# cyoq/onitama-alphazero

Hardware: AMD Instinct MI355X
Metric: MCTS node-expansions/sec/GPU @400 sims; self-play games/sec at 1/2/4/8 GPU (higher is better)
Workload: dtype fp32 (fp16x3 split)

## Files before the change

onitama-alphazero_amd/csrc/oaz_device.h:

```cpp
#pragma once

#include <stdint.h>

#include "../../include/onitama_az.h"

#if defined(__HIPCC__)
#include <hip/hip_runtime.h>
#define OAZ_HD __host__ __device__ __forceinline__
#else
#define OAZ_HD inline
#endif

namespace oaz {

constexpr uint32_t kCardPos[16] = {0x20004000u, 0x0440A000u, 0x02202000u, 0x00828000u,
                                   0x01220000u, 0x02940000u, 0x02142000u, 0x00948000u,
                                   0x0280A000u, 0x02804000u, 0x0100A000u, 0x01104000u,
                                   0x01044000u, 0x01140000u, 0x02048000u, 0x00902000u};
constexpr uint32_t kCardMir[16] = {0x01000200u, 0x02811000u, 0x02022000u, 0x00A08000u,
                                   0x00224000u, 0x0014A000u, 0x02142000u, 0x00948000u,
                                   0x0280A000u, 0x0100A000u, 0x02804000u, 0x01044000u,
                                   0x01104000u, 0x00144000u, 0x00902000u, 0x02048000u};
constexpr uint8_t kCardColor[16] = {1, 0, 0, 0, 1, 0, 1, 0, 1, 0, 1, 0, 1, 0, 1, 0};

constexpr uint32_t kRedKingStart = 0x00000200u;
constexpr uint32_t kBlueKingStart = 0x20000000u;
constexpr uint32_t kBluePawnsStart = 0xD8000000u;
constexpr uint32_t kRedPawnsStart = 0x00000D80u;
constexpr int kBlueTemple = 2;
constexpr int kRedTemple = 22;

OAZ_HD constexpr uint32_t sq_bit(int sq) { return 0x80000000u >> sq; }

struct AttackTable {
    uint32_t m[2][16][25];
};

constexpr AttackTable make_attack_table() {
    AttackTable t{};
    for (int color = 0; color < 2; ++color)
        for (int card = 0; card < 16; ++card) {
            const uint32_t pat = color ? kCardMir[card] : kCardPos[card];
            for (int from = 0; from < 25; ++from) {
                uint32_t m = 0;
                for (int j = 0; j < 25; ++j) {
                    if (!(pat & sq_bit(j))) continue;
                    const int dr = j / 5 - 2, dc = j % 5 - 2;
                    const int r = from / 5 + dr, c = from % 5 + dc;
                    if (r >= 0 && r < 5 && c >= 0 && c < 5) m |= sq_bit(r * 5 + c);
                }
                t.m[color][card][from] = m;
            }
        }
    return t;
}

constexpr AttackTable kAttackHost = make_attack_table();

OAZ_HD bool is_win(int r) { return r == OAZ_RED_WIN || r == OAZ_BLUE_WIN; }

OAZ_HD int make_move(oaz_state& s, int from, int to, int piece, int slot, int color) {
    const uint32_t fb = sq_bit(from), tb = sq_bit(to);
    const int enemy = color ^ 1;
    if (piece == OAZ_PAWN) s.pawns[color] &= ~fb;
    else s.kings[color] &= ~fb;
    int res = OAZ_IN_PROGRESS;
    if (s.pawns[enemy] & tb) {
        s.pawns[enemy] &= ~tb;
        res = OAZ_CAPTURE;
    } else if (s.kings[enemy] & tb) {
        s.kings[enemy] &= ~tb;
        res = color == OAZ_RED ? OAZ_RED_WIN : OAZ_BLUE_WIN;
    }
    if (piece == OAZ_PAWN) s.pawns[color] |= tb;
    else s.kings[color] |= tb;
    if (piece == OAZ_KING && to == (color == OAZ_RED ? kBlueTemple : kRedTemple))
        res = color == OAZ_RED ? OAZ_RED_WIN : OAZ_BLUE_WIN;
    if (slot < 4) {
        const uint8_t t = s.cards[slot];
        s.cards[slot] = s.cards[4];
        s.cards[4] = t;
    }
    return res;
}

OAZ_HD int state_card(const oaz_state& s, int i) {
    uint32_t w;
    __builtin_memcpy(&w, s.cards, 4);
    return i < 4 ? (int)((w >> (8 * i)) & 0xFFu) : (int)s.cards[4];
}
OAZ_HD void state_rotate(oaz_state& s, int slot) {
    uint32_t w;
    __builtin_memcpy(&w, s.cards, 4);
    const uint32_t sh = 8u * (uint32_t)slot;
    const uint8_t t = (uint8_t)(w >> sh);
    w = (w & ~(0xFFu << sh)) | ((uint32_t)s.cards[4] << sh);
    __builtin_memcpy(s.cards, &w, 4);
    s.cards[4] = t;
}
OAZ_HD int make_move_regs(oaz_state& s, int from, int to, int piece, int slot, int color) {
    const uint32_t fb = sq_bit(from), tb = sq_bit(to);
    const bool blue = color != OAZ_RED;
    uint32_t mp = blue ? s.pawns[1] : s.pawns[0], mk = blue ? s.kings[1] : s.kings[0];
    uint32_t ep = blue ? s.pawns[0] : s.pawns[1], ek = blue ? s.kings[0] : s.kings[1];
    if (piece == OAZ_PAWN) mp &= ~fb;
    else mk &= ~fb;
    int res = OAZ_IN_PROGRESS;
    if (ep & tb) {
        ep &= ~tb;
        res = OAZ_CAPTURE;
    } else if (ek & tb) {
        ek &= ~tb;
        res = color == OAZ_RED ? OAZ_RED_WIN : OAZ_BLUE_WIN;
    }
    if (piece == OAZ_PAWN) mp |= tb;
    else mk |= tb;
    if (piece == OAZ_KING && to == (color == OAZ_RED ? kBlueTemple : kRedTemple))
        res = color == OAZ_RED ? OAZ_RED_WIN : OAZ_BLUE_WIN;
    s.pawns[0] = blue ? ep : mp;
    s.pawns[1] = blue ? mp : ep;
    s.kings[0] = blue ? ek : mk;
    s.kings[1] = blue ? mk : ek;
    if (slot < 4) state_rotate(s, slot);
    return res;
}

OAZ_HD int current_state(const oaz_state& s) {
    if (s.kings[0] == 0 || s.kings[1] == kRedKingStart) return OAZ_BLUE_WIN;
    if (s.kings[1] == 0 || s.kings[0] == kBlueKingStart) return OAZ_RED_WIN;
    return OAZ_IN_PROGRESS;
}

OAZ_HD double reward(int result, int color) {
    if (!is_win(result)) return 0.0;
    return ((result == OAZ_RED_WIN) == (color == OAZ_RED)) ? 1.0 : -1.0;
}

OAZ_HD void initial_state(const uint8_t deck[5], oaz_state& s) {
    s.kings[0] = kRedKingStart;
    s.kings[1] = kBlueKingStart;
    s.pawns[0] = kRedPawnsStart;
    s.pawns[1] = kBluePawnsStart;
    for (int i = 0; i < 5; ++i) s.cards[i] = deck[i];
    s.to_move = kCardColor[deck[4] & 15];
    s.pad[0] = s.pad[1] = 0;
}

OAZ_HD uint16_t pack_move(int from, int to, int slot, int piece) {
    return (uint16_t)(from | (to << 5) | (slot << 10) | (piece << 12));
}
OAZ_HD int mv_from(uint32_t m) { return m & 31; }
OAZ_HD int mv_to(uint32_t m) { return (m >> 5) & 31; }
OAZ_HD int mv_slot(uint32_t m) { return (m >> 10) & 3; }
OAZ_HD int mv_piece(uint32_t m) { return (m >> 12) & 1; }

struct u32x4 {
    uint32_t x, y, z, w;
};

OAZ_HD u32x4 philox(uint64_t key, uint32_t c0, uint32_t c1, uint32_t c2, uint32_t c3) {
    uint32_t k0 = (uint32_t)key, k1 = (uint32_t)(key >> 32);
#if defined(__HIP_DEVICE_COMPILE__)
#pragma unroll
#endif
    for (int r = 0; r < 10; ++r) {
        const uint64_t p0 = (uint64_t)0xD2511F53u * c0;
        const uint64_t p1 = (uint64_t)0xCD9E8D57u * c2;
        const uint32_t n0 = (uint32_t)(p1 >> 32) ^ c1 ^ k0;
        const uint32_t n2 = (uint32_t)(p0 >> 32) ^ c3 ^ k1;
        c1 = (uint32_t)p1;
        c3 = (uint32_t)p0;
        c0 = n0;
        c2 = n2;
        k0 += 0x9E3779B9u;
        k1 += 0xBB67AE85u;
    }
    return {c0, c1, c2, c3};
}

OAZ_HD double u01(uint32_t a, uint32_t b) {
    const uint64_t m = ((uint64_t)(a >> 5) << 26) | (uint64_t)(b >> 6);
    return ((double)m + 0.5) * (1.0 / 9007199254740992.0);
}

#ifndef OAZ_NOISE_F32
#define OAZ_NOISE_F32 0
#endif
#if OAZ_NOISE_F32
typedef float noise_t;
#else
typedef double noise_t;
#endif

OAZ_HD float nz_u(uint32_t x) {
    return (float)(((x >> 9) << 1) | 1u) * (1.0f / 16777216.0f);
}
OAZ_HD float nz_log(float x) {
    uint32_t b = __builtin_bit_cast(uint32_t, x);
    int e = (int)((b >> 23) & 0xFF) - 127;
    b = (b & 0x007FFFFFu) | 0x3F800000u;
    float m = __builtin_bit_cast(float, b);
    if (m > 1.41421356f) {
        m = m * 0.5f;
        e += 1;
    }
    const float t = (m - 1.0f) / (m + 1.0f), t2 = t * t;
    const float p = t * (2.0f + t2 * (0.666666667f + t2 * (0.4f + t2 * (0.285714286f + t2 * 0.222222222f))));
    return (float)e * 0.693147182f + p;
}
OAZ_HD float nz_exp(float x) {
    if (x < -87.0f) return 0.0f;
    if (x > 88.0f) return __builtin_bit_cast(float, 0x7F800000u);
    const float k = (float)(int)(x * 1.44269504f + (x >= 0.0f ? 0.5f : -0.5f));
    const float r = (x - k * 0.693145752f) - k * 1.42860677e-6f;
    const float q = 1.0f + r * (1.0f + r * (0.5f + r * (0.166666667f + r * (0.0416666667f + r * (0.00833333333f +
                                                                                        r * 0.00138888889f)))));
    return q * __builtin_bit_cast(float, (uint32_t)((int)k + 127) << 23);
}
OAZ_HD float root_noise_f32(uint64_t seed, uint64_t game, uint32_t c2, uint32_t idx, float alpha, int K) {
    const float ia = 1.0f / alpha, ib = 1.0f / (alpha * (float)(K - 1));
    for (uint32_t t = 0; t < 1024u; ++t) {
        const u32x4 r = philox(seed, (uint32_t)game, (uint32_t)(game >> 32), c2, (idx << 12) | t);
        const float lx = nz_log(nz_u(r.x)) * ia, ly = nz_log(nz_u(r.y)) * ib;
        if (nz_exp(lx) + nz_exp(ly) <= 1.0f) return 1.0f / (1.0f + nz_exp(ly - lx));
        const float lx2 = nz_log(nz_u(r.z)) * ia, ly2 = nz_log(nz_u(r.w)) * ib;
        if (nz_exp(lx2) + nz_exp(ly2) <= 1.0f) return 1.0f / (1.0f + nz_exp(ly2 - lx2));
    }
    return 1.0f / (float)K;
}

constexpr double kLn2Hi = 6.93147180369123816490e-01, kLn2Lo = 1.90821492927058770002e-10;
OAZ_HD double nz_fma(double a, double b, double c) { return __builtin_fma(a, b, c); }
OAZ_HD double nz_log64(double x) {
    uint64_t b = __builtin_bit_cast(uint64_t, x);
    int e = (int)((b >> 52) & 0x7FF) - 1023;
    double m = __builtin_bit_cast(double, (b & 0x000FFFFFFFFFFFFFull) | 0x3FF0000000000000ull);
    if (m > 1.4142135623730951) {
        m = m * 0.5;
        e += 1;
    }
    const double t = (m - 1.0) / (m + 1.0), t2 = t * t;
    double p = 2.0 / 21.0;
    p = nz_fma(p, t2, 2.0 / 19.0);
    p = nz_fma(p, t2, 2.0 / 17.0);
    p = nz_fma(p, t2, 2.0 / 15.0);
    p = nz_fma(p, t2, 2.0 / 13.0);
    p = nz_fma(p, t2, 2.0 / 11.0);
    p = nz_fma(p, t2, 2.0 / 9.0);
    p = nz_fma(p, t2, 2.0 / 7.0);
    p = nz_fma(p, t2, 2.0 / 5.0);
    p = nz_fma(p, t2, 2.0 / 3.0);
    p = nz_fma(p * t2, t, 2.0 * t);
    const double de = (double)e;
    return nz_fma(de, kLn2Hi, nz_fma(de, kLn2Lo, p));
}
OAZ_HD double nz_exp64(double x) {
    if (x < -708.0) return 0.0;
    if (x > 709.0) return __builtin_bit_cast(double, 0x7FF0000000000000ull);
    const double k = (double)(int)(x * 1.4426950408889634 + (x >= 0.0 ? 0.5 : -0.5));
    const double r = (x - k * kLn2Hi) - k * kLn2Lo;
    double q = 1.0 / 6227020800.0;
    q = nz_fma(q, r, 1.0 / 479001600.0);
    q = nz_fma(q, r, 1.0 / 39916800.0);
    q = nz_fma(q, r, 1.0 / 3628800.0);
    q = nz_fma(q, r, 1.0 / 362880.0);
    q = nz_fma(q, r, 1.0 / 40320.0);
    q = nz_fma(q, r, 1.0 / 5040.0);
    q = nz_fma(q, r, 1.0 / 720.0);
    q = nz_fma(q, r, 1.0 / 120.0);
    q = nz_fma(q, r, 1.0 / 24.0);
    q = nz_fma(q, r, 1.0 / 6.0);
    q = nz_fma(q, r, 0.5);
    q = nz_fma(q, r, 1.0);
    q = nz_fma(q, r, 1.0);
    return q * __builtin_bit_cast(double, (uint64_t)((int64_t)k + 1023) << 52);
}
OAZ_HD double root_noise_f64(uint64_t seed, uint64_t game, uint32_t c2, uint32_t idx, double alpha, int K) {
    const double ia = 1.0 / alpha, ib = 1.0 / (alpha * (double)(K - 1));
    for (uint32_t t = 0; t < 2048u; ++t) {
        const u32x4 r = philox(seed, (uint32_t)game, (uint32_t)(game >> 32), c2, (idx << 12) | t);
        const double lx = nz_log64(u01(r.x, r.y)) * ia, ly = nz_log64(u01(r.z, r.w)) * ib;
        const double x = nz_exp64(lx), y = nz_exp64(ly), sum = x + y;
        if (sum <= 1.0) return (x > 0.0 && y > 0.0) ? x / sum : 1.0 / (1.0 + nz_exp64(ly - lx));
    }
    return 1.0 / (double)K;
}
OAZ_HD noise_t root_noise(uint64_t seed, uint64_t game, uint32_t c2, uint32_t idx, double alpha, int K) {
#if OAZ_NOISE_F32
    return root_noise_f32(seed, game, c2, idx, (float)alpha, K);
#else
    return root_noise_f64(seed, game, c2, idx, alpha, K);
#endif
}

OAZ_HD void deal_deck(uint64_t seed, uint64_t game_id, uint8_t out[5]) {
    uint8_t cards[16];
    for (int i = 0; i < 16; ++i) cards[i] = (uint8_t)i;
    uint32_t w[16];
    for (uint32_t q = 0; q < 4; ++q) {
        const u32x4 r = philox(seed, (uint32_t)game_id, (uint32_t)(game_id >> 32), 0xDEA1u, q);
        w[4 * q] = r.x;
        w[4 * q + 1] = r.y;
        w[4 * q + 2] = r.z;
        w[4 * q + 3] = r.w;
    }
    for (int i = 15, k = 0; i >= 1; --i, ++k) {
        const uint32_t j = (uint32_t)(((uint64_t)w[k] * (uint64_t)(i + 1)) >> 32);
        const uint8_t t = cards[i];
        cards[i] = cards[j];
        cards[j] = t;
    }
    for (int i = 0; i < 5; ++i) out[i] = cards[i];
}

OAZ_HD uint64_t slot_game_id(uint64_t seq, uint32_t world, uint32_t rank, uint32_t G, uint32_t g) {
    return (seq * (uint64_t)world + (uint64_t)rank) * (uint64_t)G + (uint64_t)g;
}

OAZ_HD uint64_t splitmix64(uint64_t x) {
    uint64_t z = x + 0x9E3779B97F4A7C15ull;
    z = (z ^ (z >> 30)) * 0xBF58476D1CE4E5B9ull;
    z = (z ^ (z >> 27)) * 0x94D049BB133111EBull;
    return z ^ (z >> 31);
}

OAZ_HD uint64_t hash_state(const oaz_state& s) {
    uint64_t h = splitmix64((uint64_t)s.kings[0] | ((uint64_t)s.kings[1] << 32));
    h = splitmix64(h ^ ((uint64_t)s.pawns[0] | ((uint64_t)s.pawns[1] << 32)));
    const uint64_t c = (uint64_t)(s.cards[0] & 15) | ((uint64_t)(s.cards[1] & 15) << 4) |
                       ((uint64_t)(s.cards[2] & 15) << 8) | ((uint64_t)(s.cards[3] & 15) << 12) |
                       ((uint64_t)(s.cards[4] & 15) << 16) | ((uint64_t)(s.to_move & 1) << 20);
    return splitmix64(h ^ c);
}
OAZ_HD float hash_policy(uint64_t h, int i) {
    return (float)((splitmix64(h + (uint64_t)i) >> 40) + 1) * (1.0f / 16777216.0f);
}
OAZ_HD float hash_value(uint64_t h) {
    const int32_t v = (int32_t)(splitmix64(h ^ 0x5DEECE66Dull) >> 40) - 8388608;
    return (float)v * (1.0f / 8388608.0f);
}

OAZ_HD int ab_msb_pos(uint32_t v) { return v ? 32 - __builtin_ctz(v) : 0; }
OAZ_HD int ab_distance(int from, int to) {
    const int dx = to / 5 - from / 5, dy = to % 5 - from % 5, d2 = dx * dx + dy * dy;
    return (d2 >= 1) + (d2 >= 4) + (d2 >= 9) + (d2 >= 16) + (d2 >= 25) + (d2 >= 36);
}
OAZ_HD int ab_pst_sum(uint32_t p) {
    constexpr uint32_t kRow = 0xF8000000u, kCol = 0x84210800u;
    constexpr uint32_t r13 = (kRow >> 5) | (kRow >> 15), r2 = kRow >> 10, c13 = (kCol >> 1) | (kCol >> 3), c2 = kCol >> 2;
    return 4 * (__builtin_popcount(p & r13) + 2 * __builtin_popcount(p & r2) + __builtin_popcount(p & c13) +
                2 * __builtin_popcount(p & c2));
}
OAZ_HD int32_t alphabeta_evaluate(const oaz_state& s, int color, bool won) {
    const bool blue = color != OAZ_RED;
    const int32_t sign = blue ? -1 : 1;
    if (won) return -sign * 10000;
    const uint32_t mk = blue ? s.kings[1] : s.kings[0], ek = blue ? s.kings[0] : s.kings[1];
    const uint32_t mp = blue ? s.pawns[1] : s.pawns[0], ep = blue ? s.pawns[0] : s.pawns[1];
    const int my_temple = blue ? kBlueTemple : kRedTemple, enemy_temple = blue ? kRedTemple : kBlueTemple;
    const int mkp = ab_msb_pos(mk), ekp = ab_msb_pos(ek);
    const int n_mp = __builtin_popcount(mp), n_ep = __builtin_popcount(ep);
    const uint32_t ep_seen = ep & ~mp;
    const int32_t pieces = (n_mp - n_ep) * 10 + (__builtin_popcount(mk) - __builtin_popcount(ek)) * 10000;
    const int32_t temple = ab_distance(mkp, enemy_temple) - ab_distance(ekp, my_temple);
    const int32_t close = n_mp * ab_distance(1, ekp) - __builtin_popcount(ep_seen) * ab_distance(1, mkp);
    const int32_t squares = ab_pst_sum(mp) - ab_pst_sum(ep_seen);
    return sign * (pieces + temple + close + squares);
}

OAZ_HD void random_agent_move(const AttackTable& att, uint64_t seed, uint64_t game, uint32_t ply, const oaz_state& s,
                              oaz_move& out) {
    const u32x4 r = philox(seed, (uint32_t)game, (uint32_t)(game >> 32), 0x52414E44u, ply);
    const int card_idx = (int)(((uint64_t)r.x * 2u) >> 32);
    const bool blue = (s.to_move & 1) != 0;
    const uint32_t pawns = blue ? s.pawns[1] : s.pawns[0], king = blue ? s.kings[1] : s.kings[0];
    const uint32_t own = (pawns | king) & 0xFFFFFF80u;
    const uint32_t* row = att.m[blue ? 1 : 0][state_card(s, (blue ? 2 : 0) + card_idx) & 15];
    uint32_t n = 0;
    for (uint32_t o = own; o;) {
        const int from = __builtin_clz(o);
        o &= ~sq_bit(from);
        n += (uint32_t)__builtin_popcount(row[from] & ~own);
    }
    out.from = 0;
    out.to = 5;
    out.piece = OAZ_PAWN;
    out.slot = (uint8_t)card_idx;
    if (n == 0) return;
    uint32_t k = (uint32_t)(((uint64_t)r.y * (uint64_t)n) >> 32);
    for (uint32_t o = own; o;) {
        const int from = __builtin_clz(o);
        o &= ~sq_bit(from);
        uint32_t m = row[from] & ~own;
        const uint32_t c = (uint32_t)__builtin_popcount(m);
        if (k >= c) {
            k -= c;
            continue;
        }
        for (; k; --k) m &= ~sq_bit(__builtin_clz(m));
        out.from = (uint8_t)from;
        out.to = (uint8_t)__builtin_clz(m);
        out.piece = (uint8_t)((pawns & sq_bit(from)) ? OAZ_PAWN : OAZ_KING);
        return;
    }
}

OAZ_HD int64_t total_key(double x) {
    int64_t i = (int64_t)__builtin_bit_cast(uint64_t, x);
    i ^= (int64_t)(((uint64_t)(i >> 63)) >> 1);
    return i;
}

}
```

onitama-alphazero_amd/csrc/oaz_kernels.hip:

```cpp
#include <hip/hip_runtime.h>
#include <stdlib.h>

#include <utility>

#include "oaz_device.h"
#include "oaz_kernels.h"

namespace oaz {

__constant__ AttackTable c_attack = make_attack_table();

constexpr int kWave = 64;
#ifndef OAZ_TREE_WPE
#define OAZ_TREE_WPE 8
#endif
#ifndef OAZ_TREE_WPB
#define OAZ_TREE_WPB 8
#endif
constexpr int kWavesPerBlock = OAZ_TREE_WPB;
constexpr int kBlock = kWave * kWavesPerBlock;

__device__ __forceinline__ int lane_id() { return (int)(threadIdx.x & 63); }
__device__ __forceinline__ uint32_t wave_game() {
    return blockIdx.x * kWavesPerBlock + (threadIdx.x >> 6);
}

__device__ __forceinline__ uint32_t wave_or(uint32_t v) {
#pragma unroll
    for (int off = 32; off >= 1; off >>= 1) v |= (uint32_t)__shfl_xor((int)v, off);
    return v;
}
__device__ __forceinline__ uint32_t wave_sum_u32(uint32_t v) {
#pragma unroll
    for (int off = 32; off >= 1; off >>= 1) v += (uint32_t)__shfl_xor((int)v, off);
    return v;
}
__device__ __forceinline__ uint32_t wave_max_u32(uint32_t v) {
#pragma unroll
    for (int off = 32; off >= 1; off >>= 1) v = max(v, (uint32_t)__shfl_xor((int)v, off));
    return v;
}
__device__ __forceinline__ uint32_t wave_incl_scan(uint32_t v) {
    const int l = lane_id();
#pragma unroll
    for (int off = 1; off < 64; off <<= 1) {
        const uint32_t t = (uint32_t)__shfl_up((int)v, off);
        if (l >= off) v += t;
    }
    return v;
}
__device__ __forceinline__ double readlane_f64(double v, int lane) {
    const uint64_t b = __builtin_bit_cast(uint64_t, v);
    const uint32_t lo = (uint32_t)__builtin_amdgcn_readlane((int)(uint32_t)b, lane);
    const uint32_t hi = (uint32_t)__builtin_amdgcn_readlane((int)(uint32_t)(b >> 32), lane);
    return __builtin_bit_cast(double, ((uint64_t)hi << 32) | lo);
}

__device__ __forceinline__ int wave_argmax_last(int64_t key) {
    int idx = lane_id();
#pragma unroll
    for (int off = 32; off >= 1; off >>= 1) {
        const int64_t ok = __shfl_xor(key, off);
        const int oi = __shfl_xor(idx, off);
        if (ok > key || (ok == key && oi > idx)) {
            key = ok;
            idx = oi;
        }
    }
    return idx;
}

__device__ __forceinline__ oaz_state load_state(const oaz_state* p) {
    oaz_state s;
    const uint32_t* q = reinterpret_cast<const uint32_t*>(p);
    uint32_t* d = reinterpret_cast<uint32_t*>(&s);
#pragma unroll
    for (int i = 0; i < 6; ++i) d[i] = q[i];
    return s;
}
__device__ __forceinline__ void store_state(oaz_state* p, const oaz_state& s) {
    uint32_t* q = reinterpret_cast<uint32_t*>(p);
    const uint32_t* d = reinterpret_cast<const uint32_t*>(&s);
#pragma unroll
    for (int i = 0; i < 6; ++i) q[i] = d[i];
}

struct LaneMoves {
    uint32_t mask;
    int piece;
    int slot;
    int from;
};

__device__ __forceinline__ LaneMoves lane_movegen(const oaz_state& s) {
    const int l = lane_id();
    const int color = s.to_move & 1;
    const int k = l >= 25 ? 1 : 0;
    const int from = l - 25 * k;
    const uint32_t pawns = s.pawns[color], king = s.kings[color];
    const uint32_t own = pawns | king;
    LaneMoves m;
    m.slot = (color ? 2 : 0) + k;
    m.from = from;
    m.piece = (pawns & sq_bit(from)) ? OAZ_PAWN : OAZ_KING;
    m.mask = 0;
    if (l < 50 && (own & sq_bit(from)))
        m.mask = c_attack.m[color][s.cards[m.slot] & 15][from] & ~own;
    return m;
}

__global__ void __launch_bounds__(kBlock) k_movegen(const oaz_state* __restrict__ states, int n,
                                                    uint32_t* masks, oaz_move* moves,
                                                    uint8_t* counts) {
    const uint32_t g = wave_game();
    if (g >= (uint32_t)n) return;
    const int l = lane_id();
    const oaz_state s = load_state(&states[g]);
    const LaneMoves m = lane_movegen(s);
    if (masks && l < 50) masks[(size_t)g * 50 + l] = m.mask;
    const uint32_t cnt = (uint32_t)__popc(m.mask);
    const uint32_t incl = wave_incl_scan(cnt);
    const uint32_t total = (uint32_t)__shfl((int)incl, 63);
    if (moves) {
        uint32_t o = incl - cnt, mm = m.mask;
        while (mm) {
            const int to = __clz(mm);
            mm &= ~sq_bit(to);
            if (o < OAZ_MAX_MOVES) {
                oaz_move mv;
                mv.from = (uint8_t)m.from;
                mv.to = (uint8_t)to;
                mv.piece = (uint8_t)m.piece;
                mv.slot = (uint8_t)m.slot;
                moves[(size_t)g * OAZ_MAX_MOVES + o] = mv;
            }
            ++o;
        }
        if (l < OAZ_MAX_MOVES && (uint32_t)l >= total) moves[(size_t)g * OAZ_MAX_MOVES + l] = oaz_move{0, 0, 0, 0};
    }
    if (counts && l == 0) counts[g] = (uint8_t)total;
}

__global__ void k_step(oaz_state* states, const oaz_move* mv, int n, uint8_t* results) {
    const int i = blockIdx.x * blockDim.x + threadIdx.x;
    if (i >= n) return;
    oaz_state s = states[i];
    const oaz_move m = mv[i];
    const int r = make_move(s, m.from, m.to, m.piece, m.slot, s.to_move & 1);
    s.to_move ^= 1;
    states[i] = s;
    if (results) results[i] = (uint8_t)r;
}

__global__ void k_current_state(const oaz_state* states, int n, uint8_t* results) {
    const int i = blockIdx.x * blockDim.x + threadIdx.x;
    if (i >= n) return;
    results[i] = (uint8_t)current_state(states[i]);
}

__global__ void k_encode(const oaz_state* states, int n, float* planes) {
    const long long i = (long long)blockIdx.x * blockDim.x + threadIdx.x;
    if (i >= (long long)n * 525) return;
    const int b = (int)(i / 525), r = (int)(i % 525), c = r / 25, sq = r % 25;
    const oaz_state s = states[b];
    const int color = s.to_move & 1;
    float v = 0.0f;
    if (c < 4) {
        const uint32_t src = c == 0 ? s.pawns[0] : c == 1 ? s.kings[0] : c == 2 ? s.pawns[1] : s.kings[1];
        v = (src & sq_bit(sq)) ? 1.0f : 0.0f;
    } else if (c < 20) {
        const int s0 = color ? 2 : 0;
        v = ((s.cards[s0] & 15) == c - 4 || (s.cards[s0 + 1] & 15) == c - 4) ? 1.0f : 0.0f;
    } else {
        v = color == OAZ_BLUE ? 1.0f : 0.0f;
    }
    planes[i] = v;
}

__global__ void k_hash_eval(const oaz_state* states, int n, float* policy, float* value) {
    const int i = blockIdx.x * blockDim.x + threadIdx.x;
    if (i >= n) return;
    const uint64_t h = hash_state(states[i]);
    for (int k = 0; k < 50; ++k) policy[(size_t)i * 50 + k] = hash_policy(h, k);
    value[i] = hash_value(h);
}

constexpr int kCompactThreads = (int)(kBucket / 4);
__global__ void __launch_bounds__(kCompactThreads) k_eval_compact(TreeView t) {
    __shared__ uint32_t wsum[kCompactThreads / 64];
    const uint32_t base = blockIdx.x << kBucketShift;
    const int tid = threadIdx.x, w = tid >> 6;
    const uint32_t g0 = base + 4 * (uint32_t)tid;
    oaz_state ls[4];
#pragma unroll
    for (int k = 0; k < 4; ++k) ls[k] = load_state(&t.leaf_state[g0 + k < t.G ? g0 + k : t.G - 1]);
    uint32_t f = 0;
    if (g0 + 4 <= t.G && (reinterpret_cast<uintptr_t>(t.need + g0) & 3) == 0) {
        f = *reinterpret_cast<const uint32_t*>(t.need + g0);
    } else {
#pragma unroll
        for (int k = 0; k < 4; ++k)
            if (g0 + k < t.G) f |= (uint32_t)(t.need[g0 + k] != 0) << (8 * k);
    }
    f &= 0x01010101u;
    const uint32_t cnt = (uint32_t)__popc(f);
    const uint32_t incl = wave_incl_scan(cnt);
    if (lane_id() == 63) wsum[w] = incl;
    __syncthreads();
    uint32_t off = 0, tot = 0;
#pragma unroll
    for (int i = 0; i < kCompactThreads / 64; ++i) {
        const uint32_t v = wsum[i];
        off += i < w ? v : 0u;
        tot += v;
    }
    uint32_t j = base + off + incl - cnt;
#pragma unroll
    for (int k = 0; k < 4; ++k) {
        if (f & (1u << (8 * k))) {
            const uint32_t g = g0 + k;
            t.slot[g] = j;
            store_state(&t.cstate[j], ls[k]);
            ++j;
        }
    }
    if (tid == 0) t.bcnt[blockIdx.x] = tot;
}

__global__ void __launch_bounds__(kBlock) k_root_noise(const oaz_state* __restrict__ roots,
                                                       const uint8_t* __restrict__ active,
                                                       const uint64_t* __restrict__ game_ids,
                                                       const uint32_t* __restrict__ plies, SearchParams prm,
                                                       uint32_t G, uint32_t sim0, uint32_t nsims, noise_t* out) {
    const uint32_t g = wave_game();
    if (g >= G) return;
    if (active && active[g] != 1) return;
    const int l = lane_id();
    const oaz_state s = load_state(&roots[g]);
    const LaneMoves m = lane_movegen(s);
    const int K = (int)wave_sum_u32((uint32_t)__popc(m.mask));
    if (K < 2) return;
    const uint64_t gid = game_ids ? game_ids[g] : g;
    const uint32_t ply = plies ? plies[g] : 0u;
    const int per_sim = 2 * (K - 1);
    for (int idx = l; idx < (int)nsims * per_sim; idx += 64) {
        const int k = idx / per_sim, r = idx - k * per_sim;
        const uint32_t d = 2u + (uint32_t)r;
        const uint32_t c2 = (ply << 16) | ((sim0 + k) & 0xFFFFu);
        out[((size_t)k * G + g) * kNoiseStride + d] = root_noise(prm.seed, gid, c2, d, prm.alpha, K);
    }
}

struct NodeRegs {
    double W, P;
    uint32_t N, first, misc;
};

__device__ __forceinline__ NodeRegs load_node(const oaz_node* p) {
    const uint4* q = reinterpret_cast<const uint4*>(p);
    const uint4 a = q[0], b = q[1];
    NodeRegs r;
    r.W = __builtin_bit_cast(double, ((uint64_t)a.y << 32) | a.x);
    r.P = __builtin_bit_cast(double, ((uint64_t)a.w << 32) | a.z);
    r.N = b.x;
    r.first = b.y;
    r.misc = b.z;
    return r;
}
__device__ __forceinline__ int node_nch(uint32_t misc) { return (misc >> 16) & 0xFF; }
__device__ __forceinline__ int node_flags(uint32_t misc) { return misc >> 24; }
__device__ __forceinline__ uint8_t* flags_ptr(oaz_node* n) { return &n->flags; }
__device__ __forceinline__ bool leaf_needs_eval(uint32_t misc, const oaz_state& s) {
    return !(node_flags(misc) & 3) || !is_win(current_state(s));
}

__device__ __forceinline__ void store_fresh_node(oaz_node* p, double P, uint32_t mv) {
    uint4* q = reinterpret_cast<uint4*>(p);
    const uint64_t pb = __builtin_bit_cast(uint64_t, P);
    q[0] = make_uint4(0u, 0u, (uint32_t)pb, (uint32_t)(pb >> 32));
    q[1] = make_uint4(0u, 0u, mv & 0xFFFFu, 0u);
}

__global__ void __launch_bounds__(kBlock) k_tree_reset(TreeView t) {
    const uint32_t g = blockIdx.x * blockDim.x + threadIdx.x;
    if (g >= t.G) return;
    store_fresh_node(&t.nodes[(size_t)g * t.cap], 1.0, 0);
    t.n_nodes[g] = 1;
}

__global__ void __launch_bounds__(kBlock) k_select(TreeView t, const oaz_state* __restrict__ roots,
                                                   const uint8_t* __restrict__ active,
                                                   const noise_t* __restrict__ noise,
                                                   SearchParams prm) {
    const uint32_t g = wave_game();
    if (g >= t.G) return;
    if (active && active[g] != 1) {
        if (t.need && lane_id() == 0) t.need[g] = 0;
        return;
    }
    const int l = lane_id();
    oaz_node* T = t.nodes + (size_t)g * t.cap;
    uint32_t* path = t.path + (size_t)g * t.pathcap;
    oaz_state s = load_state(&roots[g]);
    int color = s.to_move & 1;

    NodeRegs nd = load_node(&T[0]);
    uint32_t node = 0, depth = 0;
    if (l == 0) path[0] = 0;
    bool stuck = false;
    while ((node_flags(nd.misc) & 1) && !(node_flags(nd.misc) & 2)) {
        const int K = node_nch(nd.misc);
        if (K == 0) {
            stuck = true;
            break;
        }
        NodeRegs ch;
        ch.W = 0.0;
        ch.P = 0.0;
        ch.N = 0;
        ch.first = 0;
        ch.misc = 0;
        if (l < K) ch = load_node(&T[nd.first + l]);
        const double q = ch.N ? ch.W / (double)ch.N : 0.0;
        const double sq = t.sqrt_tab[nd.N] / (double)(ch.N + 1);
        int best;
        if (depth == 0 && prm.train_noise && noise) {
            double na = 0.0, nb = 0.0;
            if (l >= 1 && l < K) {
                na = (double)noise[(size_t)g * kNoiseStride + 2 * l];
                nb = (double)noise[(size_t)g * kNoiseStride + 2 * l + 1];
            }
            const double base = ch.P * (1.0 - prm.eps);
            const double ubl = q + prm.c_puct * (base + nb * prm.eps) * sq;
            int acc = 0;
            double qa = readlane_f64(q, 0), ba = readlane_f64(base, 0), sa = readlane_f64(sq, 0);
            for (int j = 1; j < K; ++j) {
                const double ua = qa + prm.c_puct * (ba + readlane_f64(na, j) * prm.eps) * sa;
                const double ub = readlane_f64(ubl, j);
                if (!(total_key(ua) > total_key(ub))) {
                    acc = j;
                    qa = readlane_f64(q, j);
                    ba = readlane_f64(base, j);
                    sa = readlane_f64(sq, j);
                }
            }
            best = acc;
        } else {
            const double u = q + prm.c_puct * ch.P * sq;
            best = wave_argmax_last(l < K ? total_key(u) : INT64_MIN);
        }
        NodeRegs c;
        c.W = __shfl(ch.W, best);
        c.P = __shfl(ch.P, best);
        c.N = (uint32_t)__shfl((int)ch.N, best);
        c.first = (uint32_t)__shfl((int)ch.first, best);
        c.misc = (uint32_t)__shfl((int)ch.misc, best);
        const uint32_t cidx = nd.first + (uint32_t)best;
        const int res = make_move(s, mv_from(c.misc), mv_to(c.misc), mv_piece(c.misc),
                                  mv_slot(c.misc), color);
        color ^= 1;
        if (is_win(res)) {
            c.misc |= 2u << 24;
            if (l == 0) *flags_ptr(&T[cidx]) = (uint8_t)(node_flags(c.misc));
        }
        ++depth;
        if (l == 0 && depth < t.pathcap) path[depth] = cidx;
        node = cidx;
        nd = c;
    }
    s.to_move = (uint8_t)color;
    if (l == 0) {
        const bool need = leaf_needs_eval(nd.misc, s);
        store_state(&t.leaf_state[g], s);
        t.leaf[g] = node;
        t.depth[g] = depth;
        if (t.need) t.need[g] = need;
        uint64_t* st = t.stats + (size_t)g * GS_COUNT;
        st[GS_SIMS] += 1;
        st[GS_DEPTH] += depth;
        st[GS_EVALS] += need;
        if (stuck) st[GS_STUCK] += 1;
    }
}

__global__ void __launch_bounds__(kBlock) k_expand_backup(TreeView t, const oaz_state* __restrict__ roots,
                                                          const uint8_t* __restrict__ active,
                                                          const float* __restrict__ policy,
                                                          const float* __restrict__ value) {
    const uint32_t g = wave_game();
    if (g >= t.G) return;
    if (active && active[g] != 1) return;
    const int l = lane_id();
    oaz_node* T = t.nodes + (size_t)g * t.cap;
    const uint32_t* path = t.path + (size_t)g * t.pathcap;
    const oaz_state s = load_state(&t.leaf_state[g]);
    const uint32_t leaf = t.leaf[g], depth = t.depth[g];
    const uint32_t row = t.slot ? t.slot[g] : g;
    const NodeRegs nd = load_node(&T[leaf]);
    uint64_t* st = t.stats + (size_t)g * GS_COUNT;
    const float* pol = policy + (size_t)row * 50;

    if (!(node_flags(nd.misc) & 3)) {
        const LaneMoves m = lane_movegen(s);
        const uint32_t cnt = (uint32_t)__popc(m.mask);
        const uint32_t incl = wave_incl_scan(cnt);
        const uint32_t K = (uint32_t)__shfl((int)incl, 63);
        const uint32_t row0 = wave_or(l < 25 ? m.mask : 0u);
        const uint32_t row1 = wave_or(l >= 25 ? m.mask : 0u);
        double sum0 = 0.0, sum1 = 0.0;
        for (int sq = 0; sq < 25; ++sq) {
            if (row0 & sq_bit(sq)) sum0 += (double)pol[sq];
            if (row1 & sq_bit(sq)) sum1 += (double)pol[25 + sq];
        }
        const uint32_t base = t.n_nodes[g];
        const int row = m.slot & 1;
        const double rs = row ? sum1 : sum0;
        uint32_t o = incl - cnt, mm = m.mask;
        while (mm) {
            const int to = __clz(mm);
            mm &= ~sq_bit(to);
            double p = (double)pol[row * 25 + to];
            if (rs > 0.0) p = p / rs;
            store_fresh_node(&T[base + o], p, pack_move(m.from, to, m.slot, m.piece));
            ++o;
        }
        if (l == 0) {
            t.n_nodes[g] = base + K;
            oaz_node* lp = &T[leaf];
            lp->first = base;
            lp->nch = (uint8_t)K;
            lp->flags = 1;
            st[GS_EXPANSIONS] += 1;
            st[GS_CHILDREN] += K;
            if (base + K > st[GS_MAXNODES]) st[GS_MAXNODES] = base + K;
        }
    }
    const int res = current_state(s);
    double r;
    if (is_win(res)) {
        const int root_color = roots[g].to_move & 1;
        const int pc = depth == 0 ? root_color : (root_color ^ (int)((depth - 1) & 1));
        r = reward(res, pc);
        if (l == 0) st[GS_TERMINAL] += 1;
    } else {
        r = (double)value[row];
    }
    const uint32_t plen = depth < t.pathcap ? depth : t.pathcap - 1;
    for (uint32_t k = (uint32_t)l; k <= plen; k += 64) {
        const uint32_t n = path[k];
        const double rk = ((depth - k) & 1) ? -r : r;
        T[n].N += 1;
        T[n].W += rk;
    }
}

constexpr int kSegLanes = 16;
__device__ __forceinline__ int seg_lane() { return (int)(threadIdx.x & 15); }
__device__ __forceinline__ int seg_base() { return (int)(threadIdx.x & 63) & ~15; }
__device__ __forceinline__ uint32_t seg_game() {
    return (blockIdx.x * kWavesPerBlock + (threadIdx.x >> 6)) * 4 + ((threadIdx.x >> 4) & 3);
}
template <int CTRL>
__device__ __forceinline__ uint32_t dpp_u32(uint32_t v) {
    return (uint32_t)__builtin_amdgcn_update_dpp(0, (int)v, CTRL, 0xF, 0xF, true);
}
template <int CTRL>
__device__ __forceinline__ void seg_amax_step(int64_t& key, int& idx) {
    const uint64_t kb = (uint64_t)key;
    const uint32_t lo = dpp_u32<CTRL>((uint32_t)kb), hi = dpp_u32<CTRL>((uint32_t)(kb >> 32));
    const int64_t ok = (int64_t)(((uint64_t)hi << 32) | lo);
    const int oi = (int)dpp_u32<CTRL>((uint32_t)idx);
    if (ok > key || (ok == key && oi > idx)) {
        key = ok;
        idx = oi;
    }
}
__device__ __forceinline__ int seg_argmax_last(int64_t key, int idx) {
    seg_amax_step<0xB1>(key, idx);
    seg_amax_step<0x4E>(key, idx);
    seg_amax_step<0x141>(key, idx);
    seg_amax_step<0x140>(key, idx);
    return idx;
}
__device__ __forceinline__ uint32_t seg_or(uint32_t v) {
    v |= dpp_u32<0xB1>(v);
    v |= dpp_u32<0x4E>(v);
    v |= dpp_u32<0x141>(v);
    v |= dpp_u32<0x140>(v);
    return v;
}
__device__ __forceinline__ uint32_t seg_incl_scan(uint32_t v) {
    v += dpp_u32<0x111>(v);
    v += dpp_u32<0x112>(v);
    v += dpp_u32<0x114>(v);
    v += dpp_u32<0x118>(v);
    return v;
}
template <class T>
__device__ __forceinline__ T pick3(int c, const T& a, const T& b, const T& d) {
    return c == 0 ? a : c == 1 ? b : d;
}

__device__ __forceinline__ void stat_add(uint64_t* p, uint64_t v) {
    (void)__hip_atomic_fetch_add(p, v, __ATOMIC_RELAXED, __HIP_MEMORY_SCOPE_AGENT);
}
__device__ __forceinline__ void stat_max(uint64_t* p, uint64_t v) {
    (void)__hip_atomic_fetch_max(p, v, __ATOMIC_RELAXED, __HIP_MEMORY_SCOPE_AGENT);
}

template <int N>
__device__ __forceinline__ double bcast_f64(double v) {
    const uint64_t b = __builtin_bit_cast(uint64_t, v);
    const uint32_t lo = (uint32_t)__builtin_amdgcn_update_dpp(0, (int)(uint32_t)b, 0x150 + N, 0xF, 0xF, true);
    const uint32_t hi = (uint32_t)__builtin_amdgcn_update_dpp(0, (int)(uint32_t)(b >> 32), 0x150 + N, 0xF, 0xF, true);
    return __builtin_bit_cast(double, ((uint64_t)hi << 32) | lo);
}
struct FoldCh {
    double q, base, sq, nae, kub;
};
__device__ __forceinline__ FoldCh fold_chunk(const NodeRegs& ch, noise_t na, noise_t nb, double sqn,
                                             const SearchParams& prm) {
    FoldCh f;
    f.q = ch.N ? ch.W / (double)ch.N : 0.0;
    f.sq = sqn / (double)(ch.N + 1);
    f.base = ch.P * (1.0 - prm.eps);
    f.nae = (double)na * prm.eps;
    const double ub = f.q + prm.c_puct * (f.base + (double)nb * prm.eps) * f.sq;
    f.kub = __builtin_bit_cast(double, total_key(ub));
    return f;
}
template <int J>
__device__ __forceinline__ void fold_step(int& acc, double& qa, double& ba, double& sa, int K, FoldCh& f,
                                          const NodeRegs (&ch)[3], const noise_t (&na)[3], const noise_t (&nb)[3],
                                          double sqn, const SearchParams& prm) {
    constexpr int c = J >> 4, n = J & 15;
    if constexpr (n == 0) f = fold_chunk(ch[c], na[c], nb[c], sqn, prm);
    const double ua = qa + prm.c_puct * (ba + bcast_f64<n>(f.nae)) * sa;
    const int64_t kb = __builtin_bit_cast(int64_t, bcast_f64<n>(f.kub));
    const double qj = bcast_f64<n>(f.q), bj = bcast_f64<n>(f.base), sj = bcast_f64<n>(f.sq);
    if (J < K && !(total_key(ua) > kb)) {
        acc = J;
        qa = qj;
        ba = bj;
        sa = sj;
    }
}
template <int... I>
__device__ __forceinline__ int root_fold(int K, int Kmax, const NodeRegs (&ch)[3], const noise_t (&na)[3],
                                         const noise_t (&nb)[3], double sqn, const SearchParams& prm,
                                         std::integer_sequence<int, I...>) {
    FoldCh f = fold_chunk(ch[0], na[0], nb[0], sqn, prm);
    int acc = 0;
// ... 809 lines not shown
```

Measured before the change: 54.18 million.

## Refill idle lanes dynamically in root noise rejection sampling

The root Dirichlet noise kernel now uses a persistent per-wave work queue. Lanes that finish their rejection-sampling draw take the next noise index through a ballot/mbcnt compaction, so no lane waits for the slowest lane's retry loop before starting new work. This targets wave divergence in the variable-length accept/reject loop, at the cost of extra ballots per iteration and more complex control flow. Output values and RNG streams stay the same.

```diff
diff --git a/onitama-alphazero_amd/csrc/oaz_device.h b/onitama-alphazero_amd/csrc/oaz_device.h
--- a/onitama-alphazero_amd/csrc/oaz_device.h
+++ b/onitama-alphazero_amd/csrc/oaz_device.h
@@ -217,15 +217,27 @@
                                                                                         r * 0.00138888889f)))));
     return q * __builtin_bit_cast(float, (uint32_t)((int)k + 127) << 23);
 }
+constexpr uint32_t kNoiseAttemptsF32 = 1024u;
+OAZ_HD bool root_noise_attempt_f32(uint64_t seed, uint64_t game, uint32_t c2, uint32_t idx, uint32_t t, float ia,
+                                   float ib, float* eta) {
+    const u32x4 r = philox(seed, (uint32_t)game, (uint32_t)(game >> 32), c2, (idx << 12) | t);
+    const float lx = nz_log(nz_u(r.x)) * ia, ly = nz_log(nz_u(r.y)) * ib;
+    if (nz_exp(lx) + nz_exp(ly) <= 1.0f) {
+        *eta = 1.0f / (1.0f + nz_exp(ly - lx));
+        return true;
+    }
+    const float lx2 = nz_log(nz_u(r.z)) * ia, ly2 = nz_log(nz_u(r.w)) * ib;
+    if (nz_exp(lx2) + nz_exp(ly2) <= 1.0f) {
+        *eta = 1.0f / (1.0f + nz_exp(ly2 - lx2));
+        return true;
+    }
+    return false;
+}
 OAZ_HD float root_noise_f32(uint64_t seed, uint64_t game, uint32_t c2, uint32_t idx, float alpha, int K) {
     const float ia = 1.0f / alpha, ib = 1.0f / (alpha * (float)(K - 1));
-    for (uint32_t t = 0; t < 1024u; ++t) {
-        const u32x4 r = philox(seed, (uint32_t)game, (uint32_t)(game >> 32), c2, (idx << 12) | t);
-        const float lx = nz_log(nz_u(r.x)) * ia, ly = nz_log(nz_u(r.y)) * ib;
-        if (nz_exp(lx) + nz_exp(ly) <= 1.0f) return 1.0f / (1.0f + nz_exp(ly - lx));
-        const float lx2 = nz_log(nz_u(r.z)) * ia, ly2 = nz_log(nz_u(r.w)) * ib;
-        if (nz_exp(lx2) + nz_exp(ly2) <= 1.0f) return 1.0f / (1.0f + nz_exp(ly2 - lx2));
-    }
+    float eta;
+    for (uint32_t t = 0; t < kNoiseAttemptsF32; ++t)
+        if (root_noise_attempt_f32(seed, game, c2, idx, t, ia, ib, &eta)) return eta;
     return 1.0f / (float)K;
 }
 
@@ -275,14 +287,21 @@
     q = nz_fma(q, r, 1.0);
     return q * __builtin_bit_cast(double, (uint64_t)((int64_t)k + 1023) << 52);
 }
+constexpr uint32_t kNoiseAttemptsF64 = 2048u;
+OAZ_HD bool root_noise_attempt_f64(uint64_t seed, uint64_t game, uint32_t c2, uint32_t idx, uint32_t t, double ia,
+                                   double ib, double* eta) {
+    const u32x4 r = philox(seed, (uint32_t)game, (uint32_t)(game >> 32), c2, (idx << 12) | t);
+    const double lx = nz_log64(u01(r.x, r.y)) * ia, ly = nz_log64(u01(r.z, r.w)) * ib;
+    const double x = nz_exp64(lx), y = nz_exp64(ly), sum = x + y;
+    if (!(sum <= 1.0)) return false;
+    *eta = (x > 0.0 && y > 0.0) ? x / sum : 1.0 / (1.0 + nz_exp64(ly - lx));
+    return true;
+}
 OAZ_HD double root_noise_f64(uint64_t seed, uint64_t game, uint32_t c2, uint32_t idx, double alpha, int K) {
     const double ia = 1.0 / alpha, ib = 1.0 / (alpha * (double)(K - 1));
-    for (uint32_t t = 0; t < 2048u; ++t) {
-        const u32x4 r = philox(seed, (uint32_t)game, (uint32_t)(game >> 32), c2, (idx << 12) | t);
-        const double lx = nz_log64(u01(r.x, r.y)) * ia, ly = nz_log64(u01(r.z, r.w)) * ib;
-        const double x = nz_exp64(lx), y = nz_exp64(ly), sum = x + y;
-        if (sum <= 1.0) return (x > 0.0 && y > 0.0) ? x / sum : 1.0 / (1.0 + nz_exp64(ly - lx));
-    }
+    double eta;
+    for (uint32_t t = 0; t < kNoiseAttemptsF64; ++t)
+        if (root_noise_attempt_f64(seed, game, c2, idx, t, ia, ib, &eta)) return eta;
     return 1.0 / (double)K;
 }
 OAZ_HD noise_t root_noise(uint64_t seed, uint64_t game, uint32_t c2, uint32_t idx, double alpha, int K) {
@@ -292,6 +311,24 @@
     return root_noise_f64(seed, game, c2, idx, alpha, K);
 #endif
 }
+struct NoiseDraw {
+    noise_t ia, ib, capped;
+    OAZ_HD NoiseDraw(double alpha, int K) {
+#if OAZ_NOISE_F32
+        ia = 1.0f / (float)alpha, ib = 1.0f / ((float)alpha * (float)(K - 1)), capped = 1.0f / (float)K;
+#else
+        ia = 1.0 / alpha, ib = 1.0 / (alpha * (double)(K - 1)), capped = 1.0 / (double)K;
+#endif
+    }
+    static constexpr uint32_t kAttempts = OAZ_NOISE_F32 ? kNoiseAttemptsF32 : kNoiseAttemptsF64;
+    OAZ_HD bool attempt(uint64_t seed, uint64_t game, uint32_t c2, uint32_t idx, uint32_t t, noise_t* eta) const {
+#if OAZ_NOISE_F32
+        return root_noise_attempt_f32(seed, game, c2, idx, t, ia, ib, eta);
+#else
+        return root_noise_attempt_f64(seed, game, c2, idx, t, ia, ib, eta);
+#endif
+    }
+};
 
 OAZ_HD void deal_deck(uint64_t seed, uint64_t game_id, uint8_t out[5]) {
     uint8_t cards[16];
diff --git a/onitama-alphazero_amd/csrc/oaz_kernels.hip b/onitama-alphazero_amd/csrc/oaz_kernels.hip
--- a/onitama-alphazero_amd/csrc/oaz_kernels.hip
+++ b/onitama-alphazero_amd/csrc/oaz_kernels.hip
@@ -235,19 +235,46 @@
     const uint32_t g = wave_game();
     if (g >= G) return;
     if (active && active[g] != 1) return;
-    const int l = lane_id();
     const oaz_state s = load_state(&roots[g]);
     const LaneMoves m = lane_movegen(s);
     const int K = (int)wave_sum_u32((uint32_t)__popc(m.mask));
     if (K < 2) return;
     const uint64_t gid = game_ids ? game_ids[g] : g;
     const uint32_t ply = plies ? plies[g] : 0u;
-    const int per_sim = 2 * (K - 1);
-    for (int idx = l; idx < (int)nsims * per_sim; idx += 64) {
-        const int k = idx / per_sim, r = idx - k * per_sim;
-        const uint32_t d = 2u + (uint32_t)r;
-        const uint32_t c2 = (ply << 16) | ((sim0 + k) & 0xFFFFu);
-        out[((size_t)k * G + g) * kNoiseStride + d] = root_noise(prm.seed, gid, c2, d, prm.alpha, K);
+    const NoiseDraw nd(prm.alpha, K);
+    const uint32_t per_sim = 2u * (uint32_t)(K - 1), total = nsims * per_sim;
+    uint32_t next = 0;
+    uint32_t d = 0, c2 = 0, t = 0;
+    size_t o = 0;
+    bool busy = false;
+    for (;;) {
+        const uint64_t idle = __ballot(!busy);
+        if (idle != 0 && next < total) {
+            const uint32_t idx = next + __builtin_amdgcn_mbcnt_hi((uint32_t)(idle >> 32),
+                                                                   __builtin_amdgcn_mbcnt_lo((uint32_t)idle, 0u));
+            if (!busy && idx < total) {
+                const uint32_t k = idx / per_sim;
+                d = 2u + (idx - k * per_sim);
+                c2 = (ply << 16) | ((sim0 + k) & 0xFFFFu);
+                o = ((size_t)k * G + g) * kNoiseStride + d;
+                t = 0;
+                busy = true;
+            }
+            next += (uint32_t)__popcll(idle);
+        }
+        if (__ballot(busy) == 0) break;
+        if (busy) {
+            noise_t eta;
+            bool done = nd.attempt(prm.seed, gid, c2, d, t, &eta);
+            if (!done && ++t == NoiseDraw::kAttempts) {
+                eta = nd.capped;
+                done = true;
+            }
+            if (done) {
+                out[o] = eta;
+                busy = false;
+            }
+        }
     }
 }
 
```

Measured after the change: 54.33 million (median of 6 runs). Within noise of the previous version (+0.3%).
